# cloudflare/zkp-ecdsa

Measured on NVIDIA H100. Metric: ZKAttest proofs/sec, higher is better.
Workload: dtype u256/u258 (32-bit limbs, Montgomery)

## Files before the change

### zkp_ecdsa_b200/csrc/zk_launch.cuh

```cuda
#pragma once
#include <stdint.h>
#include <stdlib.h>
#include <string.h>

#include <map>
#include <stdexcept>
#include <string>
#include <typeinfo>
#include <vector>

#include <cxxabi.h>

#if !defined(ZKA_HOSTSIM)
#include <cuda_runtime.h>
#endif

namespace zk {

#if !defined(ZKA_HOSTSIM)

#define ZK_CUDA_CHECK(expr)                                                                   \
  do {                                                                                        \
    cudaError_t _e = (expr);                                                                  \
    if (_e != cudaSuccess)                                                                    \
      throw std::runtime_error(std::string("CUDA error: ") + cudaGetErrorString(_e) + " at " + \
                               __FILE__ + ":" + std::to_string(__LINE__));                    \
  } while (0)

template <class Task>
struct TaskMinBlocks { static constexpr int value = 1; };

template <class Task>
__global__ void __launch_bounds__(128, TaskMinBlocks<Task>::value) zk_task_kernel(int n, Task task) {
  int t = blockIdx.x * blockDim.x + threadIdx.x;
  if (t < n) task(t);
}

struct ProfEntry {
  uint64_t launches = 0;
  double ms = 0.0;
  uint64_t items = 0;
};
struct Stream {
  cudaStream_t s = nullptr;
  uint64_t launches = 0;
  bool profiling = false;
  struct Pending { const char* name; cudaEvent_t e0, e1; long long n; };
  std::vector<Pending> pending;
  std::map<std::string, ProfEntry> prof;
};

inline std::string demangle(const char* n) {
  int status = 0;
  char* d = abi::__cxa_demangle(n, nullptr, nullptr, &status);
  std::string r = (status == 0 && d) ? d : n;
  free(d);
  return r;
}
inline void prof_collect(Stream& st) {
  for (auto& p : st.pending) {
    float ms = 0.f;
    cudaEventElapsedTime(&ms, p.e0, p.e1);
    ProfEntry& e = st.prof[demangle(p.name)];
    e.launches++;
    e.ms += ms;
    e.items += (uint64_t)p.n;
    cudaEventDestroy(p.e0);
    cudaEventDestroy(p.e1);
  }
  st.pending.clear();
}

template <class Task>
inline void launch(Stream& st, long long n, const Task& task) {
  if (n <= 0) return;
  if (n > 0x7fffffffLL) throw std::runtime_error("launch too large");
  const int threads = 128;
  const int blocks = (int)((n + threads - 1) / threads);
  Stream::Pending pd{typeid(Task).name(), nullptr, nullptr, n};
  if (st.profiling) {
    ZK_CUDA_CHECK(cudaEventCreate(&pd.e0));
    ZK_CUDA_CHECK(cudaEventCreate(&pd.e1));
    ZK_CUDA_CHECK(cudaEventRecord(pd.e0, st.s));
  }
  zk_task_kernel<Task><<<blocks, threads, 0, st.s>>>((int)n, task);
  ZK_CUDA_CHECK(cudaGetLastError());
  if (st.profiling) {
    ZK_CUDA_CHECK(cudaEventRecord(pd.e1, st.s));
    st.pending.push_back(pd);
  }
  st.launches++;
}

inline void* dev_alloc(size_t bytes) {
  void* p = nullptr;
  ZK_CUDA_CHECK(cudaMalloc(&p, bytes ? bytes : 1));
  return p;
}
inline void dev_free(void* p) {
  if (p) cudaFree(p);
}
inline void copy_h2d(Stream& st, void* d, const void* h, size_t n) {
  if (n) ZK_CUDA_CHECK(cudaMemcpyAsync(d, h, n, cudaMemcpyDefault, st.s));
}
inline void copy_d2h(Stream& st, void* h, const void* d, size_t n) {
  if (n) ZK_CUDA_CHECK(cudaMemcpyAsync(h, d, n, cudaMemcpyDefault, st.s));
}
inline void copy_d2d(Stream& st, void* d, const void* s, size_t n) {
  if (n) ZK_CUDA_CHECK(cudaMemcpyAsync(d, s, n, cudaMemcpyDeviceToDevice, st.s));
}
inline void copy_d2h_2d(Stream& st, void* h, size_t hpitch, const void* d, size_t dpitch, size_t width, size_t height) {
  if (width && height) ZK_CUDA_CHECK(cudaMemcpy2DAsync(h, hpitch, d, dpitch, width, height, cudaMemcpyDefault, st.s));
}
inline void dev_memset(Stream& st, void* d, int v, size_t n) {
  if (n) ZK_CUDA_CHECK(cudaMemsetAsync(d, v, n, st.s));
}
inline void sync(Stream& st) {
  ZK_CUDA_CHECK(cudaStreamSynchronize(st.s));
  if (!st.pending.empty()) prof_collect(st);
}
struct Event { cudaEvent_t e = nullptr; };
inline void stream_create(Stream& st) {
  if (!st.s) ZK_CUDA_CHECK(cudaStreamCreateWithFlags(&st.s, cudaStreamNonBlocking));
}
inline void stream_destroy(Stream& st) {
  if (st.s) cudaStreamDestroy(st.s);
  st.s = nullptr;
}
inline void ev_record(Event& ev, Stream& st) {
  if (!ev.e) ZK_CUDA_CHECK(cudaEventCreateWithFlags(&ev.e, cudaEventDisableTiming));
// ... 107 lines not shown
```

### zkp_ecdsa_b200/csrc/zk_ops.cuh

```cuda
#pragma once
#include "zk_curves.cuh"
#include "zk_layout.h"
#include "zk_sha256.cuh"

namespace zk {

#if defined(__CUDA_ARCH__)
#define ZK_SET_STATUS(ptr, code) atomicCAS((int*)(ptr), 0, (int)(code))
#define ZK_POST_MIN(ptr, key) atomicMin((int*)(ptr), (int)(key))
#define ZK_SET_STATUS_OVER(ptr, code, over) \
  do {                                      \
    atomicCAS((int*)(ptr), 0, (int)(code)); \
    atomicCAS((int*)(ptr), (int)(over), (int)(code)); \
  } while (0)
#else
#define ZK_SET_STATUS_OVER(ptr, code, over)              \
  do {                                                   \
    if (*(ptr) == 0 || *(ptr) == (over)) *(ptr) = (code); \
  } while (0)
#define ZK_SET_STATUS(ptr, code) \
  do {                           \
    if (*(ptr) == 0) *(ptr) = (code); \
  } while (0)
#define ZK_POST_MIN(ptr, key)             \
// ... 412 lines not shown
      const uint32_t* src = proj + (size_t)(lo + k) * TOM_PROJ_WORDS;
      uint32_t xx[9];
      tom_ld_xyz(xx, y, z, src);
      F::mul(den, y, z);
      F::mul(acc, acc, den);
      copy_n<9>(pf[k], acc);
    }
    uint32_t inv[9], s2[9], dd2[9];
    F::inv(inv, acc);
    tom_const(s2, TOM_SQRTND1);
    tom_const(dd2, TOM_2D2);
    for (int k = n - 1; k >= 0; k--) {
      const uint32_t* src = proj + (size_t)(lo + k) * TOM_PROJ_WORDS;
      uint32_t x[9], di[9], w[9], v[9], kk[9], ym[9], yp[9];
      tom_ld_xyz(x, y, z, src);
      F::mul(den, y, z);
      if (k > 0) F::mul(di, inv, pf[k - 1]); else copy_n<9>(di, inv);
      F::mul(inv, inv, den);
      F::mul(w, x, y);
      F::mul(w, w, di);
      F::mul(w, w, s2);
      F::sqr(v, z);
      F::mul(v, v, di);
      F::mul(kk, w, v);
      F::mul(kk, kk, dd2);
      F::sub(ym, v, w);
      F::add(yp, v, w);
      F::reduce(ym); F::reduce(yp); F::reduce(kk);
      uint32_t* o = pre + (size_t)(lo + k) * TOM_PRE_WORDS;
      st<9>(o, ym); st<9>(o + 9, yp); st<9>(o + 18, kk);
      for (int i = 27; i < 32; i++) o[i] = 0;
    }
  }
};

struct TomNormTask {
  const uint32_t* proj;
  uint32_t* aff;
  uint8_t* bytes;
  int count;
  int chunk;
  int e2;
  int aff_mod, aff_lim;
  int stride;
  ZK_HD static void canon2p(uint32_t* r) {
    uint32_t t[9], p2[9];
#pragma unroll
    for (int i = 0; i < 9; i++) p2[i] = (FpTom::p(i) << 1) | (i > 0 ? (FpTom::p(i - 1) >> 31) : 0u);
    uint32_t br = sub_n<9>(t, r, p2);
    csel_n<9>(r, br == 0, t, r);
    br = sub_p<FpTom>(t, r);
    csel_n<9>(r, br == 0, t, r);
  }
  ZK_HD void operator()(int t) const {
    using F = Tomp;
    const int lo = t * chunk;
    int n = count - lo;
    if (n > chunk) n = chunk;
    if (n <= 0) return;
    uint32_t pre[NORM_CHUNK_MAX][9];
    uint32_t acc[9], z[9], h[9], den[9];
    F::set_one(acc);
    for (int k = 0; k < n; k++) {
      const uint32_t* src = proj + (size_t)(lo + k) * stride;
      uint32_t xx[9], yy[9];
      if (e2) {
        tom_ld_efgh(xx, yy, z, h, src);
        F::mul(den, z, h);
      } else {
        tom_ld_xyz(xx, yy, den, src);
      }
      F::mul(acc, acc, den);
      copy_n<9>(pre[k], acc);
    }
    uint32_t inv[9], cxk[9], is2[9], one_plain[9];
    F::inv(inv, acc);
    tom_const(cxk, e2 ? TOM_INVSQRTND : TOM_INVSQRTA);
    tom_const(is2, TOM_INVSQRTND1);
    zero_n<9>(one_plain);
    one_plain[0] = 1;
    for (int k = n - 1; k >= 0; k--) {
      const uint32_t* src = proj + (size_t)(lo + k) * stride;
      uint32_t X[9], Y[9], di[9];
      if (e2) {
        tom_ld_efgh(X, Y, z, h, src);
        F::mul(den, z, h);
        F::mul(X, X, h);
        F::mul(Y, Y, z);
      } else {
        tom_ld_xyz(X, Y, den, src);
      }
      if (k > 0) F::mul(di, inv, pre[k - 1]); else copy_n<9>(di, inv);
      F::mul(inv, inv, den);
      if (bytes) {
        uint32_t Dp[9], cx[9], cy[9];
        F::mul(Dp, di, one_plain);
        F::mul(cx, X, cxk);
        F::mul(cx, cx, Dp);
        F::mul(cy, Y, Dp);
        canon2p(cx);
        canon2p(cy);
        store_point_words<9, 33>(bytes + (size_t)(lo + k) * BSTRIDE, 0x04u, cx, cy);
      }
      if (aff && ((lo + k) % aff_mod) < aff_lim) {
        uint32_t x[9], y[9];
        F::mul(x, X, di);
        if (e2) F::mul(x, x, is2);
        F::mul(y, Y, di);
        uint32_t* a = aff + (size_t)(lo + k) * TOM_AFF_WORDS;
        st<9>(a, x);
        st<9>(a + 9, y);
      }
    }
  }
};

ZK_HD void tom2_ld_entry(TomPre& q, const uint32_t* tab, const FbShape& sh, int j, uint32_t d, bool neg) {
  tom_ld_pre(q, tab + (sh.offset(j) + d) * TOM_PRE_WORDS);
  tom2_pre_neg(q, neg);
}

struct TomCommitTask {
  const uint32_t* jv;
  const uint32_t* jr;
  const uint32_t* gtab;
  const uint32_t* htab;
  uint32_t* proj;
  FbShape sh;
  int xyz = 0;
  ZK_HD void operator()(int t) const {
    uint32_t v[8], r[8];
    ld<8>(v, jv + (size_t)t * 8);
    ld<8>(r, jr + (size_t)t * 8);
    uint32_t cv = 0, cr = 0;
    bool nv, nr;
    TomPre q;
    uint32_t dv = signed_digit(v, 0, sh, cv, nv);
    tom2_ld_entry(q, gtab, sh, 0, dv, nv);
    TomPt acc;
    tom2_from_pre(acc, q);
    for (int j = 0;; j++) {
      const uint32_t dr = signed_digit(r, j, sh, cr, nr);
      tom2_ld_entry(q, htab, sh, j, dr, nr);
      if (j == sh.nwin - 1) break;
      tom2_madd<true>(acc, acc, q);
      dv = signed_digit(v, j + 1, sh, cv, nv);
      tom2_ld_entry(q, gtab, sh, j + 1, dv, nv);
      tom2_madd<true>(acc, acc, q);
    }
    if (xyz) {
      tom2_madd<false>(acc, acc, q);
      tom_st_xyz(proj + (size_t)t * TOM_PROJ_WORDS, acc.x, acc.y, acc.z);
    } else {
      TomEfgh e;
      tom2_madd_end(e, acc, q);
      tom_st_efgh(proj + (size_t)t * TOM_E2_WORDS, e);
    }
  }
};

struct TomCommitGTask {
  const uint32_t* jv;
  const uint32_t* gtab;
  uint32_t* ext;
  FbShape sh;
  ZK_HD void operator()(int t) const {
    const int item = t / GJOBS_PER_ITEM, g = t % GJOBS_PER_ITEM;
    uint32_t v[8];
    ld<8>(v, jv + ((size_t)item * JOBS_PER_ITEM + item_job_of_gpart(g)) * 8);
// ... 249 lines not shown
```

### zkp_ecdsa_b200/csrc/zk_ops_war.cuh

```cuda
#pragma once

#define WEI_PT WarPt
#define WEI_AFF WarAff
#define WEI_JAC WarJac
#define WEI_F Warp
#define WEI_FN(n) war_##n
#define WEI_T(n) War##n
#include "zk_weier_ops.inc"
#undef WEI_PT
#undef WEI_AFF
#undef WEI_JAC
#undef WEI_F
#undef WEI_FN
#undef WEI_T

struct TomNormTask {
  const uint32_t* proj;
  uint32_t* aff;
  uint8_t* bytes;
  int count;
  int chunk;
  int e2;
  int aff_mod, aff_lim;
  int stride;
  ZK_HD void operator()(int t) const {
    using F = Warp;
    const int lo = t * chunk;
    int n = count - lo;
    if (n > chunk) n = chunk;
    if (n <= 0) return;
    uint32_t pre[NORM_CHUNK_MAX][8];
    uint32_t acc[8], z[8], one[8];
    F::set_one(one);
    copy_n<8>(acc, one);
    for (int k = 0; k < n; k++) {
      ld<8>(z, proj + (size_t)(lo + k) * stride + 16);
      if (is_zero_n<8>(z)) copy_n<8>(z, one);
      F::mul(acc, acc, z);
      copy_n<8>(pre[k], acc);
    }
    uint32_t inv[8];
    F::inv(inv, acc);
    for (int k = n - 1; k >= 0; k--) {
      const uint32_t* src = proj + (size_t)(lo + k) * stride;
      ld<8>(z, src + 16);
      const bool isinf = is_zero_n<8>(z);
      if (isinf) copy_n<8>(z, one);
      uint32_t zi[8];
      if (k > 0) F::mul(zi, inv, pre[k - 1]); else copy_n<8>(zi, inv);
      F::mul(inv, inv, z);
      uint32_t X[8], Y[8], x[8], y[8];
      ld<8>(X, src);
      ld<8>(Y, src + 8);
      F::mul(x, X, zi);
      F::mul(y, Y, zi);
      if (aff && ((lo + k) % aff_mod) < aff_lim) {
        uint32_t* a = aff + (size_t)(lo + k) * TOM_AFF_WORDS;
        st<8>(a, x);
        st<8>(a + 8, y);
      }
      if (bytes) {
        uint32_t cx[8], cy[8];
        F::from_mont(cx, x);
        F::from_mont(cy, y);
        if (isinf) { zero_n<8>(cx); zero_n<8>(cy); }
        store_point_words<8, 32>(bytes + (size_t)(lo + k) * BSTRIDE, isinf ? 0x00u : 0x04u, cx, cy);
      }
    }
  }
};

struct TomCommitTask {
  const uint32_t* jv;
  const uint32_t* jr;
  const uint32_t* gtab;
  const uint32_t* htab;
  uint32_t* proj;
  FbShape sh;
  int xyz = 0;
  ZK_HD void operator()(int t) const {
    uint32_t v[8], r[8];
    ld<8>(v, jv + (size_t)t * 8);
    ld<8>(r, jr + (size_t)t * 8);
    WarJac aj;
    war_set_identity_jac(aj);
    war_accum_fixed_jac(aj, gtab, v, sh.w);
    war_accum_fixed_jac(aj, htab, r, sh.w);
    WarPt acc;
    war_jac_to_hom(acc, aj);
    war_st_proj(proj + (size_t)t * TOM_PROJ_WORDS, acc);
  }
};
struct TomCommitGTask {
  const uint32_t* jv;
  const uint32_t* gtab;
  uint32_t* ext;
  FbShape sh;
  ZK_HD void operator()(int t) const {
    const int item = t / GJOBS_PER_ITEM, g = t % GJOBS_PER_ITEM;
    uint32_t v[8];
    ld<8>(v, jv + ((size_t)item * JOBS_PER_ITEM + item_job_of_gpart(g)) * 8);
    WarJac aj;
    war_set_identity_jac(aj);
    war_accum_fixed_jac(aj, gtab, v, sh.w);
    WarPt acc;
    war_jac_to_hom(acc, aj);
    war_st_proj(ext + (size_t)t * TOM_EXT_WORDS, acc);
  }
};
struct TomCommitHTask {
  const uint32_t* jr;
  const uint32_t* htab;
  const uint32_t* ext;
  uint32_t* proj;
  FbShape sh;
  ZK_HD void operator()(int t) const {
    const int item = t / JOBS_PER_ITEM, jb = t % JOBS_PER_ITEM;
    uint32_t r[8];
    ld<8>(r, jr + (size_t)t * 8);
// ... 7 lines not shown
```

### zkp_ecdsa_b200/csrc/zk_weier_ops.inc

```
ZK_HD void WEI_FN(ld_proj)(WEI_PT& p, const uint32_t* m) {
  ld<8>(p.x, m); ld<8>(p.y, m + 8); ld<8>(p.z, m + 16);
}
ZK_HD void WEI_FN(st_proj)(uint32_t* m, const WEI_PT& p) {
  st<8>(m, p.x); st<8>(m + 8, p.y); st<8>(m + 16, p.z);
}
ZK_HD void WEI_FN(ld_aff)(WEI_AFF& a, const uint32_t* m) { ld<8>(a.x, m); ld<8>(a.y, m + 8); }
ZK_HD void WEI_FN(st_aff)(uint32_t* m, const WEI_AFF& a) { st<8>(m, a.x); st<8>(m + 8, a.y); }

struct WEI_T(PowsTask) {
  const uint32_t* base_aff;
  const uint8_t* base_inf;
  uint32_t* pows;
  int nbase, nwin, w;
  const uint32_t* index = nullptr;
  const uint32_t* count_dev = nullptr;
  const uint32_t* w_dev = nullptr;
  ZK_HD void operator()(int t) const {
    if (count_dev && (uint32_t)t >= *count_dev) return;
    const int w = w_dev ? (int)*w_dev : this->w;
    const int nwin = w_dev ? fb_windows(w) : this->nwin;
    const size_t src = index ? index[t] : (size_t)t;
    WEI_AFF a;
    WEI_FN(ld_aff)(a, base_aff + src * P256_AFF_WORDS);
    WEI_PT p;
// ... 56 lines not shown
      WEI_FN(st_proj)(out + (size_t)(blk * 16 + i) * P256_PROJ_WORDS, acc);
    }
  }
};
struct WEI_T(RowsHiTask) {
  const uint32_t* pows;
  uint32_t* hi;
  uint32_t* rows;
  int w;
  ZK_HD void operator()(int t) const {
    WEI_PT p, acc;
    WEI_FN(ld_proj)(p, pows + (size_t)t * P256_PROJ_WORDS);
    for (int k = 0; k < 8; k++) WEI_FN(dbl)(p, p);
    WEI_FN(set_identity)(acc);
    const int nh = 1 << (w - 9);
    for (int m = 0; m < nh; m++) {
      WEI_FN(st_proj)(hi + ((size_t)t * nh + m) * P256_PROJ_WORDS, acc);
      WEI_FN(add)(acc, acc, p);
    }
    WEI_FN(st_proj)(rows + ((size_t)t * fb_entries(w) + ((size_t)1 << (w - 1))) * P256_PROJ_WORDS, acc);
  }
};
struct WEI_T(RowsLoTask) {
  const uint32_t* pows;
  const uint32_t* hi;
  uint32_t* rows;
  int w;
  ZK_HD void operator()(int t) const {
    const int nh = 1 << (w - 9);
    const int j = t / nh, m = t % nh;
    WEI_PT p, acc;
    WEI_FN(ld_proj)(p, pows + (size_t)j * P256_PROJ_WORDS);
    WEI_FN(ld_proj)(acc, hi + (size_t)t * P256_PROJ_WORDS);
    uint32_t* out = rows + ((size_t)j * fb_entries(w) + ((size_t)m << 8)) * P256_PROJ_WORDS;
    for (int d = 0; d < 256; d++) {
      WEI_FN(st_proj)(out + (size_t)d * P256_PROJ_WORDS, acc);
      WEI_FN(add)(acc, acc, p);
    }
  }
};

struct WEI_T(NormTask) {
  const uint32_t* proj;
  uint32_t* aff;
  uint8_t* bytes;
  uint8_t* inf;
  int count;
  int chunk;
  const uint32_t* groups_dev = nullptr;
  int group_size = 0;
  const uint32_t* w_dev = nullptr;
  ZK_HD void operator()(int t) const {
    using F = WEI_F;
    const int lo = t * chunk;
    int total = count;
    const int group_size = w_dev ? fb_windows((int)*w_dev) * fb_entries((int)*w_dev) : this->group_size;
    if (groups_dev) {
      const long long present = (long long)*groups_dev * group_size;
      if (present < total) total = (int)present;
    }
    int n = total - lo;
    if (n > chunk) n = chunk;
    if (n <= 0) return;
    uint32_t pre[NORM_CHUNK_MAX][8];
    uint32_t acc[8], z[8], one[8];
    F::set_one(one);
    copy_n<8>(acc, one);
    for (int k = 0; k < n; k++) {
      ld<8>(z, proj + (size_t)(lo + k) * P256_PROJ_WORDS + 16);
      if (is_zero_n<8>(z)) copy_n<8>(z, one);
      F::mul(acc, acc, z);
      copy_n<8>(pre[k], acc);
    }
    uint32_t inv[8];
    F::inv(inv, acc);
    for (int k = n - 1; k >= 0; k--) {
      const uint32_t* src = proj + (size_t)(lo + k) * P256_PROJ_WORDS;
      ld<8>(z, src + 16);
      const bool isinf = is_zero_n<8>(z);
      if (isinf) copy_n<8>(z, one);
      uint32_t zi[8];
      if (k > 0) F::mul(zi, inv, pre[k - 1]); else copy_n<8>(zi, inv);
      F::mul(inv, inv, z);
      WEI_AFF a;
      uint32_t X[8], Y[8];
      ld<8>(X, src);
      ld<8>(Y, src + 8);
      F::mul(a.x, X, zi);
      F::mul(a.y, Y, zi);
      WEI_FN(st_aff)(aff + (size_t)(lo + k) * P256_AFF_WORDS, a);
      if (inf) inf[lo + k] = isinf ? 1 : 0;
      if (bytes) {
        uint8_t* o = bytes + (size_t)(lo + k) * BSTRIDE;
        uint32_t cx[8], cy[8];
        F::from_mont(cx, a.x);
        F::from_mont(cy, a.y);
        if (isinf) { zero_n<8>(cx); zero_n<8>(cy); }
        store_point_words<8, 32>(o, isinf ? 0x00u : 0x04u, cx, cy);
      }
    }
  }
};

ZK_HD void WEI_FN(accum_fixed_jac)(WEI_JAC& acc, const uint32_t* tab, const uint32_t* k, int w) {
  const int nwin = fb_windows(w);
  const size_t E = (size_t)fb_entries(w);
  uint32_t carry = 0;
  for (int j = 0; j < nwin; j++) {
    bool neg;
    const uint32_t d = signed_digit(k, j, w, carry, neg);
    if (d) {
      WEI_AFF q;
      WEI_FN(ld_aff)(q, tab + ((size_t)j * E + d) * P256_AFF_WORDS);
      if (neg) WEI_F::neg(q.y, q.y);
      WEI_FN(jac_madd)(acc, acc, q);
    }
  }
}
ZK_HD void WEI_FN(accum_fixed)(WEI_PT& acc, const uint32_t* tab, const uint32_t* k, int w) {
  WEI_JAC q;
  WEI_FN(hom_to_jac)(q, acc);
  WEI_FN(accum_fixed_jac)(q, tab, k, w);
  WEI_FN(jac_to_hom)(acc, q);
}
ZK_HD void WEI_FN(set_identity_jac)(WEI_JAC& p) {
  WEI_F::set_one(p.x);
  WEI_F::set_one(p.y);
  zero_n<8>(p.z);
}
```

### zkp_ecdsa_b200/csrc/zkattest.cu

```cuda
#include "zkattest.h"

#include <math.h>
#include <stdio.h>

#include <algorithm>
#include <atomic>
#include <cmath>
#include <mutex>
#include <chrono>
#include <memory>
#include <thread>
#include <string>
#include <vector>

#include "zk_launch.cuh"
#include "zk_prove.cuh"
#include "zk_seed.cuh"
#include "zk_verify_agg.cuh"

namespace zk {
struct ParsePointsTask {
  const uint8_t* nist;
  const uint8_t* tom;
  uint32_t* nist_aff;
// ... 171 lines not shown

ZK_HD uint64_t pack_align16(uint32_t len) { return ((uint64_t)len + 15u) & ~(uint64_t)15u; }
struct PackScanTask {
  const uint32_t* len;
  uint64_t* off;
  int B;
  ZK_HD void operator()(int) const {
    uint64_t acc = 0;
    for (int b = 0; b < B; b++) { off[b] = acc; acc += pack_align16(len[b]); }
    off[B] = acc;
  }
};
struct PackCopyTask {
  uint8_t* rows;
  size_t stride;
  const uint32_t* len;
  const uint64_t* off;
  uint8_t* packed;
  size_t cap;
  int pieces;
  int dir;
  ZK_HD void operator()(int t) const {
    const int b = t / pieces, j = t % pieces;
    const size_t o = (size_t)16 * j;
    if (o >= len[b]) return;
    const size_t po = (size_t)off[b] + o;
    if (po + 16 > cap) return;
    uint8_t* r = rows + (size_t)b * stride + o;
    uint8_t* q = packed + po;
    if (dir == 0) { for (int i = 0; i < 16; i++) q[i] = o + i < stride ? r[i] : 0; }
    else { for (int i = 0; i < 16; i++) if (o + i < stride) r[i] = q[i]; }
  }
};
struct PackCopy16Task {
  uint8_t* rows;
  size_t stride;
  const uint32_t* len;
  const uint64_t* off;
  uint8_t* packed;
  size_t cap;
  int pieces;
  int dir;
  ZK_HD void operator()(int t) const {
    const int b = t / pieces, j = t % pieces;
    const size_t o = (size_t)16 * j;
    if (o >= len[b]) return;
    const size_t po = (size_t)off[b] + o;
    if (po + 16 > cap) return;
    U4* r = reinterpret_cast<U4*>(rows + (size_t)b * stride + o);
    U4* q = reinterpret_cast<U4*>(packed + po);
    if (dir == 0) *q = *r; else *r = *q;
  }
};

}

using namespace zk;

namespace {

struct FixedTable {
  DevBuf buf;
  uint32_t* tab = nullptr;
};

}

struct Lane {
  Stream st;
  Stream cs_in, cs_out;
  Event ev_small[2], ev_tape[2], ev_done[2], ev_out[2];
  Stream aux[2];
  Event ev_fork, ev_join[2];
  DevBuf w[52];
  DevBuf in[2][10], out[2][3];
  DevBuf agg[9], agg_tom[5 + 2 * AGG_MAX_LEVELS], agg_nist[5 + 2 * AGG_MAX_LEVELS];
  std::string err;
  ~Lane() {
    for (int i = 0; i < 2; i++) {
      ev_destroy(ev_small[i]); ev_destroy(ev_tape[i]); ev_destroy(ev_done[i]); ev_destroy(ev_out[i]);
    }
    ev_destroy(ev_fork); ev_destroy(ev_join[0]); ev_destroy(ev_join[1]);
    stream_destroy(cs_in);
    stream_destroy(cs_out);
    stream_destroy(aux[0]);
    stream_destroy(aux[1]);
    stream_destroy(st);
  }
};

struct zka_ctx : Lane {
  int device = 0;
  std::vector<std::unique_ptr<Lane>> extra;
  int nlanes = 3;
  DevBuf ring_in, ring_m;
  DevBuf ring_leaves, ring_digest;
  Lane& lane(int i) { return i == 0 ? *this : *extra[i - 1]; }
#if defined(ZKA_PG_WAR256)
  FbShape tom = fb_uniform(22);
#else
  FbShape tom = fb_lookups(11);
#endif
  size_t tom_table_max = 0;
  bool tom_fallback = false;
  int chunk = 4096;
  int host_chunk = 2048;
// ... 39 lines not shown
namespace {

int fail(zka_ctx* ctx, int code, const std::string& msg) {
  if (ctx) ctx->err = msg;
  return code;
}
template <class Fn>
int guarded(zka_ctx* ctx, Fn&& body) {
  try {
    return body();
  } catch (const std::exception& e) {
    return fail(ctx, ZKA_E_CUDA, e.what());
  }
}

template <class Src>
void agg_msm(Stream& st, Cursor A, const Src& src, const AggPlan& pl, const uint32_t* ctl, const uint32_t** rootA,
             const uint32_t** rootB) {
  const AggDigits& D = pl.D;
  const int nwin = D.nwin, nb = D.nb, nseg = (nb + 1 + AGG_SEG - 1) / AGG_SEG;
  const size_t cap = (size_t)src.slots();
  uint32_t* hist = A.take<uint32_t>((size_t)nwin * (nb + 1));
  uint32_t* bstart = A.take<uint32_t>((size_t)nwin * (nb + 2));
  uint32_t* segtot = A.take<uint32_t>((size_t)nwin * nseg);
  uint32_t* sorted = A.take<uint32_t>((size_t)nwin * cap);
  uint32_t* bsum = A.take<uint32_t>((size_t)nwin * nb * Src::PTW);
  dev_memset(st, hist, 0, (size_t)nwin * (nb + 1) * 4);
  launch(st, (long long)cap, AggHistTask<Src>{src, D, ctl, hist});
  launch(st, (long long)nwin * nseg, AggSegSumTask{ctl, hist, segtot, nb, nseg});
  launch(st, nwin, AggSegScanTask{ctl, segtot, nseg});
  launch(st, (long long)nwin * nseg, AggOffsetsTask{ctl, segtot, hist, bstart, nb, nseg});
  launch(st, (long long)cap, AggScatterTask<Src>{src, D, ctl, hist, sorted, cap});
  launch(st, (long long)nwin * nb, AggBucketTask<Src>{src, ctl, bstart, sorted, bsum, cap, nb});
  const uint32_t *inA = bsum, *inB = nullptr;
  int nin = nb, ll = 0;
  for (int lv = 0; lv < pl.levels; lv++) {
    const int nout = nin >> pl.lm[lv];
    uint32_t* oA = A.take<uint32_t>((size_t)nwin * nout * Src::PTW);
    uint32_t* oB = A.take<uint32_t>((size_t)nwin * nout * Src::PTW);
    launch(st, (long long)nwin * nout, AggLevelTask<Src>{ctl, inA, inB, oA, oB, nin, pl.lm[lv], ll, nwin, D.top_shift});
    inA = oA; inB = oB; nin = nout; ll += pl.lm[lv];
  }
  *rootA = inA;
  *rootB = inB;
}

int ceil_log2(uint32_t v) {
  int n = 0;
  while ((1ull << n) < v) n++;
  return n;
}


static int g_norm_slots = 132 * 4;
static bool g_norm_model = true;
inline int norm_chunk_for(long long count, int per_point = 11) {
  if (!g_norm_model) {
    long long c = count / 100000;
    if (c < 8) c = 8;
    if (c > NORM_CHUNK_MAX) c = NORM_CHUNK_MAX;
    return (int)c;
  }
  int best = 8;
  long long best_cost = -1;
  for (int c = 8; c <= NORM_CHUNK_MAX; c++) {
    const long long threads = (count + c - 1) / c, ctas = (threads + 127) / 128;
    const long long waves = (ctas + g_norm_slots - 1) / g_norm_slots;
    const long long cost = waves * ((long long)per_point * c + 70);
    if (best_cost < 0 || cost < best_cost) { best_cost = cost; best = c; }
  }
  return best;
}
inline void launch_p256_norm(Stream& st, const uint32_t* proj, uint32_t* aff, uint8_t* bytes, uint8_t* inf, long long count) {
  if (count <= 0) return;
  const int ch = norm_chunk_for(count, bytes ? 7 : 5);
  launch(st, (count + ch - 1) / ch, P256NormTask{proj, aff, bytes, inf, (int)count, ch});
}
inline void launch_tom_norm(Stream& st, const uint32_t* proj, uint32_t* aff, uint8_t* bytes, long long count, int e2,
                            int aff_mod = 1, int aff_lim = 1, int stride = 0) {
  if (count <= 0) return;
  const int ch = norm_chunk_for(count);
  if (stride == 0) stride = e2 ? TOM_E2_WORDS : TOM_PROJ_WORDS;
  launch(st, (count + ch - 1) / ch, TomNormTask{proj, aff, bytes, (int)count, ch, e2, aff_mod, aff_lim, stride});
}

void build_p256_tab(zka_ctx* ctx, const uint32_t* base_aff_dev, FixedTable& out, int w) {
  Stream& st = ctx->st;
  const int nwin = fb_windows(w);
  const size_t E = (size_t)fb_entries(w), count = (size_t)nwin * E;
  DevBuf pows, rows;
  uint32_t* d_pows = pows.get<uint32_t>((size_t)nwin * P256_PROJ_WORDS);
  uint32_t* d_rows = rows.get<uint32_t>(count * P256_PROJ_WORDS);
  out.tab = out.buf.get<uint32_t>(count * P256_AFF_WORDS);
  launch(st, 1, P256PowsTask{base_aff_dev, nullptr, d_pows, 1, nwin, w});
  if (w > 9) {
    DevBuf hi;
    const int nh = 1 << (w - 9);
    uint32_t* d_hi = hi.get<uint32_t>((size_t)nwin * nh * P256_PROJ_WORDS);
    launch(st, nwin, P256RowsHiTask{d_pows, d_hi, d_rows, w});
    launch(st, (long long)nwin * nh, P256RowsLoTask{d_pows, d_hi, d_rows, w});
    sync(st);
  } else {
    launch(st, nwin, P256RowsTask{d_pows, d_rows, w});
  }
  launch_p256_norm(st, d_rows, out.tab, nullptr, nullptr, (long long)(count));
  sync(st);
}
uint32_t* alloc_tom_tab(zka_ctx* ctx, DevBuf& buf) {
  const size_t words = ctx->tom.total() * TOM_PRE_WORDS;
  if (ctx->tom_table_max && words * sizeof(uint32_t) > ctx->tom_table_max)
    throw std::runtime_error("proof-group fixed-base table of " + std::to_string(words * sizeof(uint32_t)) + " bytes exceeds ZKA_TOM_TABLE_MAX");
  return buf.get_exact<uint32_t>(words);
}
#if defined(ZKA_PG_WAR256)
void build_tom_tab(zka_ctx* ctx, const uint32_t* base_aff_dev, FixedTable& out) {
  Stream& st = ctx->st;
  const int w = ctx->tom.w, nwin = ctx->tom.nwin;
  const size_t E = (size_t)fb_entries(w), count = (size_t)nwin * E;
  DevBuf pows, rows;
  uint32_t* d_pows = pows.get<uint32_t>((size_t)nwin * P256_PROJ_WORDS);
  uint32_t* d_rows = rows.get<uint32_t>(count * P256_PROJ_WORDS);
  out.tab = alloc_tom_tab(ctx, out.buf);
  launch(st, 1, WarPowsTask{base_aff_dev, nullptr, d_pows, 1, nwin, w});
  if (w > 9) {
    DevBuf hi;
    const int nh = 1 << (w - 9);
    uint32_t* d_hi = hi.get<uint32_t>((size_t)nwin * nh * P256_PROJ_WORDS);
    launch(st, nwin, WarRowsHiTask{d_pows, d_hi, d_rows, w});
    launch(st, (long long)nwin * nh, WarRowsLoTask{d_pows, d_hi, d_rows, w});
    sync(st);
  } else {
    launch(st, nwin, WarRowsTask{d_pows, d_rows, w});
  }
  {
    const int ch = norm_chunk_for((long long)count, 5);
    launch(st, ((long long)count + ch - 1) / ch, WarNormTask{d_rows, out.tab, nullptr, nullptr, (int)count, ch});
  }
  sync(st);
}
#else
void build_tom_tab(zka_ctx* ctx, const uint32_t* base_aff_dev, FixedTable& out) {
  Stream& st = ctx->st;
  const FbShape sh = ctx->tom;
  out.tab = alloc_tom_tab(ctx, out.buf);
  DevBuf pows, rows, hi;
  uint32_t* d_pows = pows.get<uint32_t>((size_t)sh.nwin * 36);
  uint32_t* d_rows = rows.get<uint32_t>(sh.entries(sh.nwin - 1) * TOM_PROJ_WORDS);
  launch(st, 1, TomPowsTask{base_aff_dev, d_pows, 1, sh});
  const bool two_level = sh.w > 9;
  uint32_t* d_hi = nullptr;
  if (two_level) {
    d_hi = hi.get<uint32_t>(tom_hi_offset(sh, sh.nwin) * 36);
    launch(st, sh.nwin, TomRowsHiTask{d_pows, d_hi, sh});
  }
  for (int j = 0; j < sh.nwin; j++) {
    const size_t ne = sh.entries(j);
    const uint32_t* pw = d_pows + (size_t)j * 36;
    if (two_level) {
      const int nh = 1 << (sh.width(j) - 9);
      launch(st, nh + 1, TomRowsLoTask{pw, d_hi + tom_hi_offset(sh, j) * 36, d_rows, nh});
    } else {
      launch(st, 1, TomRowsTask{pw, d_rows, sh.width(j)});
    }
    launch(st, (long long)(ne + 15) / 16, TomTabE2Task{d_rows, out.tab + sh.offset(j) * TOM_PRE_WORDS, (int)ne});
  }
  sync(st);
}

#endif

template <class T>
const T* stage_in(Stream& st, DevBuf& buf, const T* p, size_t count) {
  if (!p || count == 0) return p;
  if (is_device_ptr(p)) return p;
  T* d = buf.get<T>(count);
  copy_h2d(st, d, p, count * sizeof(T));
  return d;
}

template <class T>
struct Output {
  T* dst;
  size_t width;
  bool dev;
  Output(T* p, size_t width) : dst(p), width(width), dev(is_device_ptr(p)) {}
  T* rows(DevBuf& stage, uint32_t b0, size_t rows) const { return dev ? dst + b0 * width : stage.get<T>(rows * width); }
  void copy_back(Stream& st, uint32_t b0, const T* d, size_t rows) const {
    if (!dev) copy_d2h(st, dst + b0 * width, d, rows * width * sizeof(T));
// ... 377 lines not shown
  const std::vector<uint32_t> v = chunk_schedule(B, (uint32_t)(host_buffers ? std::min(ctx->chunk, ctx->host_chunk) : ctx->chunk), ctx->nlanes,
                                                 host_buffers != 0);
  if (v.size() > cap) return ZKA_E_ARG;
  for (size_t i = 0; i < v.size(); i++) off[i] = v[i];
  return (int)v.size() - 1;
}
int zka_lanes(const zka_ctx* ctx) { return ctx ? ctx->nlanes : 0; }
int zka_config(const zka_ctx* ctx, int* tom_w, int* tom_nwin, int* chunk) {
  if (!ctx) return ZKA_E_ARG;
  if (tom_w) *tom_w = ctx->tom.w;
  if (tom_nwin) *tom_nwin = ctx->tom.nwin;
  if (chunk) *chunk = ctx->chunk;
  return 0;
}

int zka_init(int device, zka_ctx** out) {
  if (!out) return ZKA_E_ARG;
  *out = nullptr;
#if !defined(ZKA_HOSTSIM)
  int ndev = 0;
  cudaError_t e = cudaGetDeviceCount(&ndev);
  if (e != cudaSuccess || ndev == 0 || device >= ndev) {
    cudaGetLastError();
    return ZKA_E_CUDA;
  }
#endif
  std::unique_ptr<zka_ctx> ctx(new zka_ctx());
  const int rc = guarded(ctx.get(), [&] {
#if !defined(ZKA_HOSTSIM)
    ZK_CUDA_CHECK(cudaSetDevice(device));
    ZK_CUDA_CHECK(cudaStreamCreateWithFlags(&ctx->st.s, cudaStreamNonBlocking));
#endif
    ctx->device = device;
    [[maybe_unused]] bool tom_pinned = false;
    if (const char* e = getenv("ZKA_TOM_W")) {
      int w = atoi(e);
      if (w >= 2 && w <= 24) { ctx->tom = fb_uniform(w); tom_pinned = true; }
    }
#if !defined(ZKA_PG_WAR256)
    if (const char* e = tom_pinned ? nullptr : getenv("ZKA_TOM_NWIN")) {
      int n = atoi(e);
      if (n >= 11 && n <= 128) ctx->tom = fb_lookups(n);
    }
#endif
    if (const char* e = getenv("ZKA_TOM_TABLE_MAX")) ctx->tom_table_max = (size_t)strtoull(e, nullptr, 10);
    if (const char* e = getenv("ZKA_CHUNK")) {
      int c = atoi(e);
      if (c >= 1) ctx->chunk = c;
    }
    if (const char* e = getenv("ZKA_NORM_MODEL")) g_norm_model = atoi(e) != 0;
#if !defined(ZKA_HOSTSIM)
    {
      int sms = 0;
      if (cudaDeviceGetAttribute(&sms, cudaDevAttrMultiProcessorCount, device) == cudaSuccess && sms > 0) g_norm_slots = sms * 4;
    }
#endif
    if (const char* e = getenv("ZKA_HOST_CHUNK")) {
      int c = atoi(e);
      if (c >= 1) ctx->host_chunk = c;
    }
    stream_create(ctx->cs_in);
    stream_create(ctx->cs_out);
    stream_create(ctx->aux[0]);
    stream_create(ctx->aux[1]);
    {
      int lanes = 3;
#if defined(ZKA_HOSTSIM)
      lanes = 1;
#endif
      if (const char* e = getenv("ZKA_LANES")) lanes = atoi(e);
      if (lanes < 1) lanes = 1;
      if (lanes > 8) lanes = 8;
      if (zka_set_option(ctx.get(), "lanes", lanes) != 0) throw std::runtime_error("lanes");
    }
    if (const char* e = getenv("ZKA_TAPE_SPLIT")) ctx->tape_split = atoi(e) != 0;
    if (const char* e = getenv("ZKA_AGG")) ctx->agg = atoi(e);
    if (const char* e = getenv("ZKA_AGG_C")) {
      int c = atoi(e);
      if (c >= 4 && c <= 16) ctx->agg_c = c;
    }
    if (const char* e = getenv("ZKA_P256_HW")) {
      int w = atoi(e);
      if (w >= 8 && w <= 24) ctx->p256_hw = w;
    }
    DevBuf gen;
    uint32_t* d_gen = gen.get<uint32_t>(16 + TOM_AFF_WORDS);
    launch(ctx->st, 1, GenAffTask{d_gen, d_gen + 16});
    build_p256_tab(ctx.get(), d_gen, ctx->g8, 8);
    build_p256_tab(ctx.get(), d_gen, ctx->gw, ctx->p256_hw);
#if defined(ZKA_PG_WAR256)
    build_tom_tab(ctx.get(), d_gen + 16, ctx->tg);
#else
    try {
      DevBuf room;
      alloc_tom_tab(ctx.get(), room);
      build_tom_tab(ctx.get(), d_gen + 16, ctx->tg);
    } catch (const std::exception&) {
      if (tom_pinned || ctx->tom.nwin >= 128) throw;
#if !defined(ZKA_HOSTSIM)
      cudaGetLastError();
#endif
      ctx->tg.buf.release();
      ctx->tom = fb_lookups(ctx->tom.nwin + 1);
      ctx->tom_fallback = true;
      build_tom_tab(ctx.get(), d_gen + 16, ctx->tg);
    }
#endif
// ... 372 lines not shown
      c.r_bytes = w.take<uint8_t>((size_t)Bc * BSTRIDE);
      c.rpows = w.take<uint32_t>((size_t)Bc * RT_NWIN * P256_PROJ_WORDS);
      c.rrows = w.take<uint32_t>((size_t)Bc * KEY_CAP * P256_PROJ_WORDS);
      c.rtab = w.take<uint32_t>((size_t)Bc * KEY_CAP * P256_AFF_WORDS);
      c.pa_T = w.take<uint32_t>(nA * P256_PROJ_WORDS);
      c.pa_A = w.take<uint32_t>(nA * P256_PROJ_WORDS);
      c.pa_T_aff = w.take<uint32_t>(nA * 16);
      c.pa_T_inf = w.take<uint8_t>(nA);
      c.pa_A_aff = w.take<uint32_t>(nA * 16);
      c.pa_A_bytes = w.take<uint8_t>(nA * BSTRIDE);
      c.pa_A_inf = w.take<uint8_t>(nA);
      c.s1_jv = w.take<uint32_t>(n1 * 8);
      c.s1_jr = w.take<uint32_t>(n1 * 8);
      c.s1_proj = w.take<uint32_t>(n1 * TOM_E2_WORDS);
      c.s1_aff = w.take<uint32_t>(n1 * TOM_AFF_WORDS);
      c.s1_bytes = w.take<uint8_t>(n1 * BSTRIDE);
      c.chal = w.take<uint32_t>((size_t)Bc * 3);
      c.zcount = w.take<uint32_t>(Bc);
      c.item_base = w.take<uint32_t>(Bc);
      c.item_total = w.take<uint32_t>(2);
      c.rep_off = w.take<uint32_t>((size_t)Bc * S);
      c.gk_off = w.take<uint32_t>(Bc);
      c.gk_dv = w.take<uint32_t>((size_t)Bc * n * 8);
      c.gk_x = w.take<uint32_t>((size_t)Bc * 3);
      c.u12 = w.take<uint32_t>((size_t)Bc * 16);
      c.tab_of = w.take<uint32_t>(Bc);
      c.tab_rep = w.take<uint32_t>((size_t)Bc * 2);
      c.tab_count = w.take<uint32_t>(2);
      c.which_s = w.take<uint32_t>(Bc);
      uint32_t* base_aff = w.take_if<uint32_t>(mode == 1, (size_t)Bc * 16);
      c.base_aff = mode == 0 ? c.pk_aff : base_aff;
      uint8_t* hedged = w.take_if<uint8_t>(hedge, (size_t)Bc * 32);
      const uint8_t* seeds = hedge ? hedged : cin[slot].seeds;
      c.proof_stride = rows.proof_stride;
      Cursor ob(ln.out[slot]);
      c.proofs = po.rows(ob.next(), b0, Bc);
      c.proof_len = lo.rows(ob.next(), b0, Bc);
      c.status = so.rows(ob.next(), b0, Bc);

      launch(st, Bc, PreKeyTask{c});
      launch(st, Bc, KeyDedupTask{c});
      launch(st, Bc, KeyRankTask{c});
      launch(st, Bc, KeyAssignTask{c});
      {
        const int Bp = (Bc + 31) & ~31;
        launch(st, (long long)Bp + Bc,
               PowsAndPreTask{P256PowsTask{c.base_aff, nullptr, c.rpows, Bc, RT_NWIN, RT_W, c.tab_rep, c.tab_count, c.tab_count + 1}, PreTask{c}, Bp});
      }
      launch(st, (long long)Bc * ((KEY_CAP + 15) / 16), P256RowsBlockTask{c.rpows, c.rrows, KEY_W_MIN, c.tab_count, c.tab_count + 1});
      {
        const long long np = (long long)Bc * KEY_CAP;
        const uint32_t kest = ring.set ? (uint32_t)Bc : std::min<uint32_t>(ring.N, (uint32_t)Bc);
        const int west = key_window_bits(kest, (uint32_t)Bc, (uint32_t)S + 2);
        const int ch = norm_chunk_for((long long)kest * fb_windows(west) * fb_entries(west), 5);
        launch(st, (np + ch - 1) / ch, P256NormTask{c.rrows, c.rtab, nullptr, nullptr, (int)np, ch, c.tab_count, 0, c.tab_count + 1});
      }
      ev_wait(st, ln.ev_tape[slot]);
      if (hedge) {
        SeedHedgeTask ht{{}, ring_digest, cin[slot].ring_of, cin[slot].seeds, c.msg_hash, c.sig, c.pk, c.which, hedged};
        memcpy(ht.params_digest, P->hedge_digest, 32);
        launch(st, Bc, ht);
      }
      if (seeded) {
        const int d1 = draws_before_items(S);
        launch(st, (long long)Bc * d1, SeedProveTapeTask{seeds, const_cast<uint8_t*>(c.tape), c.tape_stride, S, n, 0, d1, nullptr});
      }
      {
        const int nAp = (int)((nA + 31) & ~(size_t)31);
        launch(st, (long long)nAp + Bc, PhaseAAndRPointTask{PhaseAP256Task{c}, RPointTask{c}, (int)nA, nAp});
      }
      launch_p256_norm(st, c.pa_T, c.pa_T_aff, nullptr, c.pa_T_inf, (long long)(nA));
      launch_p256_norm(st, c.pa_A, c.pa_A_aff, c.pa_A_bytes, c.pa_A_inf, (long long)(nA));
      if (mode == 1) launch(st, Bc, ExpStatementTask{c});
      prove_store1(st, c);
      launch(st, Bc, ExpChallengeTask{c});
      launch(st, 1, ScanTask{c});
      uint32_t tot2[2] = {0, 0};
      copy_d2h(st, tot2, c.item_total, 8);
      const bool tape_host = !seeded && ctx->tape_split && !is_device_ptr(rows.tape);
      sync(st);
      if (seeded) {
        const int d1 = draws_before_items(S), span = prove_draws((int)tot2[1], n, S) - d1;
        launch(st, (long long)Bc * span,
               SeedProveTapeTask{seeds, const_cast<uint8_t*>(c.tape), c.tape_stride, S, n, d1, span, c.zcount, c.ring_of, c.ring_depth});
      } else if (tape_host) {
        const size_t o0 = (size_t)32 * draws_before_items(S);
        const size_t o1 = std::min(rows.tape_stride, (size_t)32 * prove_draws((int)tot2[1], n, S));
        if (o1 > o0)
          copy_d2h_2d(st, const_cast<uint8_t*>(c.tape) + o0, c.tape_stride, rows.at(b0).tape + o0, rows.tape_stride, o1 - o0, Bc);
      }
      const double t_mid = ms_now();
      {
        const uint32_t kn = next_chunk.fetch_add(1);
        if (kn < nchunks) issue_inputs(kn, slot ^ 1);
        k = kn;
      }
      const uint32_t M = tot2[0];
      const size_t max_len = mode == 0 ? (size_t)proof_len((int)tot2[1], n, S)
                                       : (size_t)tot2[1] * REP0_LEN + (size_t)(S - (int)tot2[1]) * REP1_LEN;
      c.M = (int)M;
      c.item_b = w.take<uint32_t>(M);
      c.item_i = w.take<uint32_t>(M);
      c.item_k = w.take<uint32_t>(M);
      c.pb_T1 = w.take<uint32_t>((size_t)M * P256_PROJ_WORDS);
      c.pb_T1_aff = w.take<uint32_t>((size_t)M * 16);
      c.pb_T1_inf = w.take<uint8_t>(M);
      const size_t n2 = c.s2_count();
// ... 878 lines not shown
```

Before: 118,700.

## Stride-interleave batched-inversion norm kernels, prefetch denominators, tune occupancy per task

Each thread of the normalization kernels now walks points spaced T apart instead of a contiguous chunk, so neighbouring threads touch neighbouring rows and loads coalesce. The next denominator is prefetched with vector loads. The Tom kernel drops redundant multiplies and stores per-factor prefix products. Per-task launch-bounds min-blocks and an occupancy-derived slot count feed a per-task chunk cost model. Raising min blocks can force register spills, and the doubled prefix array raises local memory use.

```diff
diff --git a/zkp_ecdsa_b200/csrc/zk_launch.cuh b/zkp_ecdsa_b200/csrc/zk_launch.cuh
--- a/zkp_ecdsa_b200/csrc/zk_launch.cuh
+++ b/zkp_ecdsa_b200/csrc/zk_launch.cuh
@@ -16,6 +16,8 @@
 #endif
 
 namespace zk {
+
+constexpr int TASK_THREADS = 128;
 
 #if !defined(ZKA_HOSTSIM)
 
@@ -31,7 +33,7 @@
 struct TaskMinBlocks { static constexpr int value = 1; };
 
 template <class Task>
-__global__ void __launch_bounds__(128, TaskMinBlocks<Task>::value) zk_task_kernel(int n, Task task) {
+__global__ void __launch_bounds__(TASK_THREADS, TaskMinBlocks<Task>::value) zk_task_kernel(int n, Task task) {
   int t = blockIdx.x * blockDim.x + threadIdx.x;
   if (t < n) task(t);
 }
@@ -75,7 +77,7 @@
 inline void launch(Stream& st, long long n, const Task& task) {
   if (n <= 0) return;
   if (n > 0x7fffffffLL) throw std::runtime_error("launch too large");
-  const int threads = 128;
+  const int threads = TASK_THREADS;
   const int blocks = (int)((n + threads - 1) / threads);
   Stream::Pending pd{typeid(Task).name(), nullptr, nullptr, n};
   if (st.profiling) {
diff --git a/zkp_ecdsa_b200/csrc/zk_ops.cuh b/zkp_ecdsa_b200/csrc/zk_ops.cuh
--- a/zkp_ecdsa_b200/csrc/zk_ops.cuh
+++ b/zkp_ecdsa_b200/csrc/zk_ops.cuh
@@ -488,69 +488,102 @@
     br = sub_p<FpTom>(t, r);
     csel_n<9>(r, br == 0, t, r);
   }
+  ZK_HD void ld_den_words(uint32_t* w, int i) const {
+    const uint32_t* s = proj + (size_t)i * stride + 16;
+#pragma unroll
+    for (int j = 0; j < 5; j++)
+      if (j < 3 || e2) ld4(w + 4 * j, s + 4 * j);
+  }
+  ZK_HD static void ld_rr(uint32_t* r) {
+#pragma unroll
+    for (int i = 0; i < 9; i++) r[i] = FpTom::rr(i);
+  }
+  ZK_HD void ld_head_words(uint32_t* w, int i) const {
+    const uint32_t* s = proj + (size_t)i * stride;
+#pragma unroll
+    for (int j = 0; j < 4; j++) ld4(w + 4 * j, s + 4 * j);
+  }
   ZK_HD void operator()(int t) const {
     using F = Tomp;
-    const int lo = t * chunk;
-    int n = count - lo;
-    if (n > chunk) n = chunk;
-    if (n <= 0) return;
-    uint32_t pre[NORM_CHUNK_MAX][9];
-    uint32_t acc[9], z[9], h[9], den[9];
+    const int T = (count + chunk - 1) / chunk;
+    if (t >= T) return;
+    const int n = (count - t + T - 1) / T;
+    uint32_t pre[2 * NORM_CHUNK_MAX][9];
+    uint32_t acc[9], nw[20];
+    zero_n<20>(nw);
     F::set_one(acc);
+    ld_den_words(nw, t);
+    int m = 0;
     for (int k = 0; k < n; k++) {
-      const uint32_t* src = proj + (size_t)(lo + k) * stride;
-      uint32_t xx[9], yy[9];
+      uint32_t w[20];
+      copy_n<20>(w, nw);
+      if (k + 1 < n) ld_den_words(nw, t + (k + 1) * T);
+      F::mul(acc, acc, w + 2);
+      copy_n<9>(pre[m++], acc);
       if (e2) {
-        tom_ld_efgh(xx, yy, z, h, src);
-        F::mul(den, z, h);
+        F::mul(acc, acc, w + 11);
+        copy_n<9>(pre[m++], acc);
+      }
+    }
+    uint32_t inv[9], cxk[9], xk[9];
+    F::inv(inv, acc);
+    {
+      uint32_t one_plain[9];
+      zero_n<9>(one_plain);
+      one_plain[0] = 1;
+      F::mul(inv, inv, one_plain);
+    }
+    tom_const(cxk, e2 ? TOM_INVSQRTND : TOM_INVSQRTA);
+    ld_rr(xk);
+    if (aff && e2) {
+      uint32_t is2[9];
+      tom_const(is2, TOM_INVSQRTND1);
+      F::mul(xk, is2, xk);
+    }
+    ld_den_words(nw, t + (n - 1) * T);
+    for (int k = n - 1; k >= 0; k--) {
+      const int i = t + k * T;
+      uint32_t w[36];
+      ld_head_words(w, i);
+      copy_n<20>(w + 16, nw);
+      if (k > 0) ld_den_words(nw, i - T);
+      uint32_t dx[9], dy[9];
+      m--;
+      if (m > 0) F::mul(dy, inv, pre[m - 1]); else copy_n<9>(dy, inv);
+      F::mul(inv, inv, e2 ? w + 27 : w + 18);
+      if (e2) {
+        m--;
+        if (m > 0) F::mul(dx, inv, pre[m - 1]); else copy_n<9>(dx, inv);
+        F::mul(inv, inv, w + 18);
       } else {
-        tom_ld_xyz(xx, yy, den, src);
+        copy_n<9>(dx, dy);
       }
-      F::mul(acc, acc, den);
-      copy_n<9>(pre[k], acc);
-    }
-    uint32_t inv[9], cxk[9], is2[9], one_plain[9];
-    F::inv(inv, acc);
-    tom_const(cxk, e2 ? TOM_INVSQRTND : TOM_INVSQRTA);
-    tom_const(is2, TOM_INVSQRTND1);
-    zero_n<9>(one_plain);
-    one_plain[0] = 1;
-    for (int k = n - 1; k >= 0; k--) {
-      const uint32_t* src = proj + (size_t)(lo + k) * stride;
-      uint32_t X[9], Y[9], di[9];
-      if (e2) {
-        tom_ld_efgh(X, Y, z, h, src);
-        F::mul(den, z, h);
-        F::mul(X, X, h);
-        F::mul(Y, Y, z);
-      } else {
-        tom_ld_xyz(X, Y, den, src);
-      }
-      if (k > 0) F::mul(di, inv, pre[k - 1]); else copy_n<9>(di, inv);
-      F::mul(inv, inv, den);
+      const uint32_t* X = w;
+      const uint32_t* Y = w + 9;
+      uint32_t cy[9];
       if (bytes) {
-        uint32_t Dp[9], cx[9], cy[9];
-        F::mul(Dp, di, one_plain);
+        uint32_t cx[9];
         F::mul(cx, X, cxk);
-        F::mul(cx, cx, Dp);
-        F::mul(cy, Y, Dp);
+        F::mul(cx, cx, dx);
+        F::mul(cy, Y, dy);
         canon2p(cx);
         canon2p(cy);
-        store_point_words<9, 33>(bytes + (size_t)(lo + k) * BSTRIDE, 0x04u, cx, cy);
+        store_point_words<9, 33>(bytes + (size_t)i * BSTRIDE, 0x04u, cx, cy);
       }
-      if (aff && ((lo + k) % aff_mod) < aff_lim) {
+      if (aff && (i % aff_mod) < aff_lim) {
         uint32_t x[9], y[9];
-        F::mul(x, X, di);
-        if (e2) F::mul(x, x, is2);
-        F::mul(y, Y, di);
-        uint32_t* a = aff + (size_t)(lo + k) * TOM_AFF_WORDS;
+        F::mul(x, X, dx);
+        F::mul(x, x, xk);
+        if (!bytes) F::mul(cy, Y, dy);
+        ld_rr(y);
+        F::mul(y, cy, y);
+        uint32_t* a = aff + (size_t)i * TOM_AFF_WORDS;
         st<9>(a, x);
         st<9>(a + 9, y);
       }
     }
   }
 };
-
 ZK_HD void tom2_ld_entry(TomPre& q, const uint32_t* tab, const FbShape& sh, int j, uint32_t d, bool neg) {
   tom_ld_pre(q, tab + (sh.offset(j) + d) * TOM_PRE_WORDS);
   tom2_pre_neg(q, neg);
diff --git a/zkp_ecdsa_b200/csrc/zk_ops_war.cuh b/zkp_ecdsa_b200/csrc/zk_ops_war.cuh
--- a/zkp_ecdsa_b200/csrc/zk_ops_war.cuh
+++ b/zkp_ecdsa_b200/csrc/zk_ops_war.cuh
@@ -25,16 +25,18 @@
   int stride;
   ZK_HD void operator()(int t) const {
     using F = Warp;
-    const int lo = t * chunk;
-    int n = count - lo;
-    if (n > chunk) n = chunk;
-    if (n <= 0) return;
+    const int T = (count + chunk - 1) / chunk;
+    if (t >= T) return;
+    const int n = (count - t + T - 1) / T;
     uint32_t pre[NORM_CHUNK_MAX][8];
-    uint32_t acc[8], z[8], one[8];
+    uint32_t acc[8], one[8], nz[8];
     F::set_one(one);
     copy_n<8>(acc, one);
+    ld8v(nz, proj + (size_t)t * stride + 16);
     for (int k = 0; k < n; k++) {
-      ld<8>(z, proj + (size_t)(lo + k) * stride + 16);
+      uint32_t z[8];
+      copy_n<8>(z, nz);
+      if (k + 1 < n) ld8v(nz, proj + (size_t)(t + (k + 1) * T) * stride + 16);
       if (is_zero_n<8>(z)) copy_n<8>(z, one);
       F::mul(acc, acc, z);
       copy_n<8>(pre[k], acc);
@@ -42,20 +44,22 @@
     uint32_t inv[8];
     F::inv(inv, acc);
     for (int k = n - 1; k >= 0; k--) {
-      const uint32_t* src = proj + (size_t)(lo + k) * stride;
-      ld<8>(z, src + 16);
+      const int i = t + k * T;
+      const uint32_t* src = proj + (size_t)i * stride;
+      uint32_t X[8], Y[8], z[8];
+      ld8v(z, src + 16);
+      ld8v(X, src);
+      ld8v(Y, src + 8);
       const bool isinf = is_zero_n<8>(z);
       if (isinf) copy_n<8>(z, one);
       uint32_t zi[8];
       if (k > 0) F::mul(zi, inv, pre[k - 1]); else copy_n<8>(zi, inv);
       F::mul(inv, inv, z);
-      uint32_t X[8], Y[8], x[8], y[8];
-      ld<8>(X, src);
-      ld<8>(Y, src + 8);
+      uint32_t x[8], y[8];
       F::mul(x, X, zi);
       F::mul(y, Y, zi);
-      if (aff && ((lo + k) % aff_mod) < aff_lim) {
-        uint32_t* a = aff + (size_t)(lo + k) * TOM_AFF_WORDS;
+      if (aff && (i % aff_mod) < aff_lim) {
+        uint32_t* a = aff + (size_t)i * TOM_AFF_WORDS;
         st<8>(a, x);
         st<8>(a + 8, y);
       }
@@ -64,7 +68,7 @@
         F::from_mont(cx, x);
         F::from_mont(cy, y);
         if (isinf) { zero_n<8>(cx); zero_n<8>(cy); }
-        store_point_words<8, 32>(bytes + (size_t)(lo + k) * BSTRIDE, isinf ? 0x00u : 0x04u, cx, cy);
+        store_point_words<8, 32>(bytes + (size_t)i * BSTRIDE, isinf ? 0x00u : 0x04u, cx, cy);
       }
     }
   }
diff --git a/zkp_ecdsa_b200/csrc/zk_weier_ops.inc b/zkp_ecdsa_b200/csrc/zk_weier_ops.inc
--- a/zkp_ecdsa_b200/csrc/zk_weier_ops.inc
+++ b/zkp_ecdsa_b200/csrc/zk_weier_ops.inc
@@ -132,22 +132,24 @@
   const uint32_t* w_dev = nullptr;
   ZK_HD void operator()(int t) const {
     using F = WEI_F;
-    const int lo = t * chunk;
     int total = count;
     const int group_size = w_dev ? fb_windows((int)*w_dev) * fb_entries((int)*w_dev) : this->group_size;
     if (groups_dev) {
       const long long present = (long long)*groups_dev * group_size;
       if (present < total) total = (int)present;
     }
-    int n = total - lo;
-    if (n > chunk) n = chunk;
-    if (n <= 0) return;
+    const int T = (total + chunk - 1) / chunk;
+    if (t >= T) return;
+    const int n = (total - t + T - 1) / T;
     uint32_t pre[NORM_CHUNK_MAX][8];
-    uint32_t acc[8], z[8], one[8];
+    uint32_t acc[8], one[8], nz[8];
     F::set_one(one);
     copy_n<8>(acc, one);
+    ld8v(nz, proj + (size_t)t * P256_PROJ_WORDS + 16);
     for (int k = 0; k < n; k++) {
-      ld<8>(z, proj + (size_t)(lo + k) * P256_PROJ_WORDS + 16);
+      uint32_t z[8];
+      copy_n<8>(z, nz);
+      if (k + 1 < n) ld8v(nz, proj + (size_t)(t + (k + 1) * T) * P256_PROJ_WORDS + 16);
       if (is_zero_n<8>(z)) copy_n<8>(z, one);
       F::mul(acc, acc, z);
       copy_n<8>(pre[k], acc);
@@ -155,23 +157,24 @@
     uint32_t inv[8];
     F::inv(inv, acc);
     for (int k = n - 1; k >= 0; k--) {
-      const uint32_t* src = proj + (size_t)(lo + k) * P256_PROJ_WORDS;
-      ld<8>(z, src + 16);
+      const int i = t + k * T;
+      const uint32_t* src = proj + (size_t)i * P256_PROJ_WORDS;
+      uint32_t X[8], Y[8], z[8];
+      ld8v(z, src + 16);
+      ld8v(X, src);
+      ld8v(Y, src + 8);
       const bool isinf = is_zero_n<8>(z);
       if (isinf) copy_n<8>(z, one);
       uint32_t zi[8];
       if (k > 0) F::mul(zi, inv, pre[k - 1]); else copy_n<8>(zi, inv);
       F::mul(inv, inv, z);
       WEI_AFF a;
-      uint32_t X[8], Y[8];
-      ld<8>(X, src);
-      ld<8>(Y, src + 8);
       F::mul(a.x, X, zi);
       F::mul(a.y, Y, zi);
-      WEI_FN(st_aff)(aff + (size_t)(lo + k) * P256_AFF_WORDS, a);
-      if (inf) inf[lo + k] = isinf ? 1 : 0;
+      WEI_FN(st_aff)(aff + (size_t)i * P256_AFF_WORDS, a);
+      if (inf) inf[i] = isinf ? 1 : 0;
       if (bytes) {
-        uint8_t* o = bytes + (size_t)(lo + k) * BSTRIDE;
+        uint8_t* o = bytes + (size_t)i * BSTRIDE;
         uint32_t cx[8], cy[8];
         F::from_mont(cx, a.x);
         F::from_mont(cy, a.y);
diff --git a/zkp_ecdsa_b200/csrc/zkattest.cu b/zkp_ecdsa_b200/csrc/zkattest.cu
--- a/zkp_ecdsa_b200/csrc/zkattest.cu
+++ b/zkp_ecdsa_b200/csrc/zkattest.cu
@@ -247,6 +247,13 @@
     if (dir == 0) *q = *r; else *r = *q;
   }
 };
+
+#if !defined(ZKA_HOSTSIM) && !defined(ZKA_PG_WAR256)
+template <> struct TaskMinBlocks<TomNormTask> { static constexpr int value = 4; };
+template <> struct TaskMinBlocks<P256NormTask> { static constexpr int value = 6; };
+#elif !defined(ZKA_HOSTSIM)
+template <> struct TaskMinBlocks<P256NormTask> { static constexpr int value = 6; };
+#endif
 
 }
 
@@ -392,20 +399,31 @@
 }
 
 
-static int g_norm_slots = 132 * 4;
+template <class Task>
+int g_norm_slots = 132 * 4;
 static bool g_norm_model = true;
-inline int norm_chunk_for(long long count, int per_point = 11) {
+#if !defined(ZKA_HOSTSIM)
+template <class Task>
+void read_norm_slots(int sms) {
+  int ctas = 0;
+  if (cudaOccupancyMaxActiveBlocksPerMultiprocessor(&ctas, zk_task_kernel<Task>, TASK_THREADS, 0) == cudaSuccess && ctas > 0)
+    g_norm_slots<Task> = sms * ctas;
+}
+#endif
+template <class Task>
+int norm_chunk_for(long long count, int per_point) {
   if (!g_norm_model) {
     long long c = count / 100000;
     if (c < 8) c = 8;
     if (c > NORM_CHUNK_MAX) c = NORM_CHUNK_MAX;
     return (int)c;
   }
+  const int slots = g_norm_slots<Task>;
   int best = 8;
   long long best_cost = -1;
   for (int c = 8; c <= NORM_CHUNK_MAX; c++) {
-    const long long threads = (count + c - 1) / c, ctas = (threads + 127) / 128;
-    const long long waves = (ctas + g_norm_slots - 1) / g_norm_slots;
+    const long long threads = (count + c - 1) / c, ctas = (threads + TASK_THREADS - 1) / TASK_THREADS;
+    const long long waves = (ctas + slots - 1) / slots;
     const long long cost = waves * ((long long)per_point * c + 70);
     if (best_cost < 0 || cost < best_cost) { best_cost = cost; best = c; }
   }
@@ -413,13 +431,18 @@
 }
 inline void launch_p256_norm(Stream& st, const uint32_t* proj, uint32_t* aff, uint8_t* bytes, uint8_t* inf, long long count) {
   if (count <= 0) return;
-  const int ch = norm_chunk_for(count, bytes ? 7 : 5);
+  const int ch = norm_chunk_for<P256NormTask>(count, bytes ? 7 : 5);
   launch(st, (count + ch - 1) / ch, P256NormTask{proj, aff, bytes, inf, (int)count, ch});
 }
 inline void launch_tom_norm(Stream& st, const uint32_t* proj, uint32_t* aff, uint8_t* bytes, long long count, int e2,
                             int aff_mod = 1, int aff_lim = 1, int stride = 0) {
   if (count <= 0) return;
-  const int ch = norm_chunk_for(count);
+#if defined(ZKA_PG_WAR256)
+  const int per_point = 5 + (bytes ? 2 : 0);
+#else
+  const int per_point = (e2 ? 6 : 3) + (bytes ? 3 : 0) + (aff ? (bytes ? 3 : 4) * aff_lim / aff_mod : 0);
+#endif
+  const int ch = norm_chunk_for<TomNormTask>(count, per_point);
   if (stride == 0) stride = e2 ? TOM_E2_WORDS : TOM_PROJ_WORDS;
   launch(st, (count + ch - 1) / ch, TomNormTask{proj, aff, bytes, (int)count, ch, e2, aff_mod, aff_lim, stride});
 }
@@ -473,7 +496,7 @@
     launch(st, nwin, WarRowsTask{d_pows, d_rows, w});
   }
   {
-    const int ch = norm_chunk_for((long long)count, 5);
+    const int ch = norm_chunk_for<WarNormTask>((long long)count, 5);
     launch(st, ((long long)count + ch - 1) / ch, WarNormTask{d_rows, out.tab, nullptr, nullptr, (int)count, ch});
   }
   sync(st);
@@ -957,7 +980,13 @@
 #if !defined(ZKA_HOSTSIM)
     {
       int sms = 0;
-      if (cudaDeviceGetAttribute(&sms, cudaDevAttrMultiProcessorCount, device) == cudaSuccess && sms > 0) g_norm_slots = sms * 4;
+      if (cudaDeviceGetAttribute(&sms, cudaDevAttrMultiProcessorCount, device) == cudaSuccess && sms > 0) {
+        read_norm_slots<TomNormTask>(sms);
+        read_norm_slots<P256NormTask>(sms);
+#if defined(ZKA_PG_WAR256)
+        read_norm_slots<WarNormTask>(sms);
+#endif
+      }
     }
 #endif
     if (const char* e = getenv("ZKA_HOST_CHUNK")) {
@@ -1436,7 +1465,7 @@
         const long long np = (long long)Bc * KEY_CAP;
         const uint32_t kest = ring.set ? (uint32_t)Bc : std::min<uint32_t>(ring.N, (uint32_t)Bc);
         const int west = key_window_bits(kest, (uint32_t)Bc, (uint32_t)S + 2);
-        const int ch = norm_chunk_for((long long)kest * fb_windows(west) * fb_entries(west), 5);
+        const int ch = norm_chunk_for<P256NormTask>((long long)kest * fb_windows(west) * fb_entries(west), 5);
         launch(st, (np + ch - 1) / ch, P256NormTask{c.rrows, c.rtab, nullptr, nullptr, (int)np, ch, c.tab_count, 0, c.tab_count + 1});
       }
       ev_wait(st, ln.ev_tape[slot]);
```

Result: no change. 119,200, median of 6 (+0.4%).
